# linto-ai/ssak

Hardware: AMD Instinct MI355X
Metric: utterances/sec (16 kHz, 10 s) Wav2Vec2-base CTC train step (higher is better)
Workload: dtype bf16; 1 GPU; Wav2Vec2-base CTC fine-tune step, bf16, synthetic 10 s @16 kHz utterances (BASELINE.json configs[1]; DP over xGMI for n_gpus>1 = configs[2]); per_gpu_batch=32, global_batch=32, samples_per_utt=160000, frames=499, frozen_feature_encoder=True, regularisers=script defaults (dropout/layerdrop/specaugment on), parallelism=dp1

## Files before the change

### ssak_amd/csrc/attention.hip

```cpp
#include <utility>

#include "kernels.h"

namespace {

constexpr int HD = 64;
constexpr int KT = 64;
constexpr int TILE = 2;
constexpr int TILE_BYTES = KT * HD * 2;
typedef __attribute__((address_space(3))) void lds_void_t;
typedef __attribute__((address_space(3))) s16x4 lds_s16x4_t;
typedef __attribute__((ext_vector_type(8))) short s16x8_t;
typedef __attribute__((ext_vector_type(4))) uint32_t u32x4_t;

struct AttnParams {
  const bf16* qkv;
  bf16* ctx;
  float* lse;
  const int32_t* klens;
  const bf16* dctx;
  float* delta;
  bf16* dqkv;
  float* bias_part;
  int B, F, nh, H, Fp;
  float scale;
  uint64_t seed;
  uint32_t stream, thresh16;
  float drop_scale;
};

__device__ __forceinline__ float shfl_xor_f(float v, int m) { return __shfl_xor(v, m, 64); }
__device__ __forceinline__ float softmax_offset(float v, float slack) {
  float x = v, y = v;
  asm volatile("s_nop 1\n\tv_permlane16_swap_b32 %0, %1" : "+v"(x), "+v"(y));
  float pm;
  asm("v_max_f32 %0, %1, %2" : "=v"(pm) : "v"(x), "v"(y));
  float a = pm, b = pm;
  asm volatile("s_nop 1\n\tv_permlane32_swap_b32 %0, %1" : "+v"(a), "+v"(b));
  float all;
  asm("v_max_f32 %0, %1, %2" : "=v"(all) : "v"(a), "v"(b));
  float g0 = x, g2 = x;
  asm volatile("s_nop 1\n\tv_permlane32_swap_b32 %0, %1" : "+v"(g0), "+v"(g2));
  float r;
  asm("v_max_f32 %0, %1, %2" : "=v"(r) : "v"(g0), "v"(all - slack));
  return r;
}
__device__ __forceinline__ float max2_nc(float a, float b) {
  float d;
  asm("v_max_f32 %0, %1, %2" : "=v"(d) : "v"(a), "v"(b));
  return d;
}
__device__ __forceinline__ float max3_nc(float a, float b, float c) {
  float d;
  asm("v_max3_f32 %0, %1, %2, %3" : "=v"(d) : "v"(a), "v"(b), "v"(c));
  return d;
}
__device__ __forceinline__ int opaque_s(int v) {
  asm volatile("" : "+s"(v));
  return v;
}

__device__ __forceinline__ uint32_t drop_rowseed(const AttnParams& p, int b, int h, int q) {
  return drop_rowkey(p.seed, p.stream, (uint64_t)((uint32_t)(b * p.nh + h) * (uint32_t)p.F + (uint32_t)min(q, p.F - 1)));
}
__device__ __forceinline__ void fill_colmul(uint32_t* cmt, int n) {
  for (int k = threadIdx.x; k < n; k += 256) cmt[k] = drop_colmul((uint32_t)k);
}

#ifdef ATT_OLD_DUAL
__device__ __forceinline__ int dual_swz(int r) {
  const int x = (r >> 1) & 7;
  return ((x << 1) & 7) | (x >> 2);
}
#else
__device__ __forceinline__ int dual_swz(int r) { return r & 6; }
#endif
__device__ __forceinline__ void dma_tile(__amdgpu_buffer_rsrc_t rsrc, char* lds_tile, uint32_t col_byte, long ld_bytes,
                                         int row0, int nrows_total, int image , int wave, int lane) {
#pragma unroll
  for (int j = 0; j < 2; ++j) {
    const int S = (wave * 2 + j) * 64 + lane;
    const int r = S >> 3, pc = S & 7;
    const int c = image == 2 ? (pc ^ dual_swz(r)) : image == 1 ? (pc ^ (r & 6)) : (pc ^ ((r >> 1) & 7));
    const int gr = row0 + r;
    const uint32_t off = gr < nrows_total ? (uint32_t)((long)gr * ld_bytes + col_byte + c * 16) : 0x80000000u;
    __builtin_amdgcn_raw_ptr_buffer_load_lds(rsrc, (lds_void_t*)(lds_tile + (wave * 2 + j) * 1024), 16, off, 0, 0, 0);
  }
}

struct DmaOff {
  uint32_t o[2];
};
__device__ __forceinline__ DmaOff dma_offsets(uint32_t col_byte, long ld_bytes, int image, int wave, int lane) {
  DmaOff d;
#pragma unroll
  for (int j = 0; j < 2; ++j) {
    const int S = (wave * 2 + j) * 64 + lane;
    const int r = S >> 3, pc = S & 7;
    const int c = image == 2 ? (pc ^ dual_swz(r)) : image == 1 ? (pc ^ (r & 6)) : (pc ^ ((r >> 1) & 7));
    d.o[j] = (uint32_t)((long)r * ld_bytes + col_byte + c * 16);
  }
  return d;
}
__device__ __forceinline__ __amdgpu_buffer_rsrc_t rsrc_rows(const void* base, long ld_bytes, int row0, int nrows) {
  const long skip = (long)row0 * ld_bytes;
  return __builtin_amdgcn_make_buffer_rsrc((void*)((const char*)base + skip), 0, (int)((long)max(nrows - row0, 0) * ld_bytes), 0x00020000);
}
__device__ __forceinline__ void dma_tile_at(__amdgpu_buffer_rsrc_t rsrc, char* lds_tile, const DmaOff& d, int wave) {
#pragma unroll
  for (int j = 0; j < 2; ++j)
    __builtin_amdgcn_raw_ptr_buffer_load_lds(rsrc, (lds_void_t*)(lds_tile + (wave * 2 + j) * 1024), 16, d.o[j], 0, 0, 0);
}

__device__ __forceinline__ bf16x8 frag_rows(const char* tile, int sub, int kk, int lane) {
  const int r = 16 * sub + (lane & 15);
  const int c = kk * 4 + (lane >> 4);
  return *reinterpret_cast<const bf16x8*>(tile + r * 128 + ((c ^ ((r >> 1) & 7)) << 4));
}
__device__ __forceinline__ bf16x8 frag_cols_perm(const char* tile, int ci, int rbase, int lane) {
  const int g = lane >> 4, q4 = (lane >> 2) & 3, p4 = lane & 3;
  const int r = rbase + 4 * g + q4;
  const int ch = 2 * ci + (p4 >> 1);
  const char* a = tile + r * 128 + ((ch ^ (r & 6)) << 4) + (p4 & 1) * 8;
  const s16x4 lo = __builtin_amdgcn_ds_read_tr16_b64_v4i16((lds_s16x4_t*)(a));
  const s16x4 hi = __builtin_amdgcn_ds_read_tr16_b64_v4i16((lds_s16x4_t*)(a + 16 * 128));
  s16x8_t v = __builtin_shufflevector(lo, hi, 0, 1, 2, 3, 4, 5, 6, 7);
  return __builtin_bit_cast(bf16x8, v);
}

__device__ __forceinline__ bf16x8 frag_rows_d(const char* tile, int sub, int kk, int lane) {
  const int r = 16 * sub + (lane & 15);
  const int c = kk * 4 + (lane >> 4);
  return *reinterpret_cast<const bf16x8*>(tile + r * 128 + ((c ^ dual_swz(r)) << 4));
}
__device__ __forceinline__ bf16x8 frag_cols_perm_d(const char* tile, int ci, int rbase, int lane) {
  const int g = lane >> 4, q4 = (lane >> 2) & 3, p4 = lane & 3;
  const int r = rbase + 4 * g + q4;
  const int ch = 2 * ci + (p4 >> 1);
  const char* a = tile + r * 128 + ((ch ^ dual_swz(r)) << 4) + (p4 & 1) * 8;
  const s16x4 lo = __builtin_amdgcn_ds_read_tr16_b64_v4i16((lds_s16x4_t*)(a));
  const s16x4 hi = __builtin_amdgcn_ds_read_tr16_b64_v4i16((lds_s16x4_t*)(a + 16 * 128));
  s16x8_t v = __builtin_shufflevector(lo, hi, 0, 1, 2, 3, 4, 5, 6, 7);
  return __builtin_bit_cast(bf16x8, v);
}

__device__ __forceinline__ bf16x8 pack_p(const f32x4& a, const f32x4& b) {
  const bf16x4 lo = __builtin_convertvector(a, bf16x4), hi = __builtin_convertvector(b, bf16x4);
  return __builtin_shufflevector(lo, hi, 0, 1, 2, 3, 4, 5, 6, 7);
}

__device__ __forceinline__ bf16x8 load_row_frag(const bf16* base, long ld, int row, int nrows, int kk, int lane) {
  bf16x8 z = {};
  if (row >= nrows) return z;
  return *reinterpret_cast<const bf16x8*>(base + (long)row * ld + 32 * kk + 8 * (lane >> 4));
}

struct AttnBlock {
  int b, h, blk;
};
__device__ __forceinline__ AttnBlock attn_block() {
  const int nblk = gridDim.x, nh = gridDim.y, nbh = gridDim.y * gridDim.z;
  AttnBlock r;
  if ((nbh & 7) != 0) {
    r.b = blockIdx.z, r.h = blockIdx.y, r.blk = blockIdx.x;
    return r;
  }
  const int L = blockIdx.x + nblk * (blockIdx.y + nh * blockIdx.z);
  const int xcd = L & 7, j = L >> 3;
  const int bh = (j / nblk) * 8 + xcd;
  r.blk = j % nblk;
  r.b = bh / nh;
  r.h = bh % nh;
  return r;
}

template <int NS>
__device__ __forceinline__ void bias_partial(float (&cs)[NS][4][4], char* smem, float* dst , int set_stride,
                                             int wave, int lane) {
#pragma unroll
  for (int s = 0; s < NS; ++s)
#pragma unroll
    for (int i = 0; i < 4; ++i)
#pragma unroll
      for (int r = 0; r < 4; ++r) {
        float v = cs[s][i][r];
        v += dpp_f<0xB1, 0xf>(0.f, v);
        v += dpp_f<0x4E, 0xf>(0.f, v);
        v += dpp_f<0x141, 0xf>(0.f, v);
        v += dpp_f<0x140, 0xf>(0.f, v);
        cs[s][i][r] = v;
      }
  float* red = reinterpret_cast<float*>(smem);
  lds_barrier();
  if ((lane & 15) == 0) {
#pragma unroll
    for (int s = 0; s < NS; ++s)
#pragma unroll
      for (int i = 0; i < 4; ++i)
        *reinterpret_cast<f32x4*>(red + (s * 4 + wave) * HD + 16 * i + 4 * (lane >> 4)) = (f32x4){cs[s][i][0], cs[s][i][1], cs[s][i][2], cs[s][i][3]};
  }
  lds_barrier();
  if (wave < NS) {
    const float* rs = red + wave * 4 * HD;
    dst[wave * set_stride + lane] = (rs[lane] + rs[HD + lane]) + (rs[2 * HD + lane] + rs[3 * HD + lane]);
  }
}
__device__ __forceinline__ float bf16_round(float v) { return (float)(bf16)v; }

typedef __attribute__((ext_vector_type(2))) float f32x2;

template <bool DROP, int NQS>
__global__ __launch_bounds__(256) void attn_fwd_kernel(const AttnParams p) {
  extern __shared__ __attribute__((aligned(16))) char smem[];
  const int lane = threadIdx.x & 63, wave = __builtin_amdgcn_readfirstlane(threadIdx.x >> 6);
  const AttnBlock ab = attn_block();
  const int b = ab.b, h = ab.h, q0 = ab.blk * (64 * NQS);
  const int F = p.F, H = p.H;
  const long ld = 3L * H;
  const bf16* base = p.qkv + (long)b * F * ld;
  const int kl = p.klens ? min(max(p.klens[b], 0), F) : F;
  const int nkt = (kl + KT - 1) / KT;
  __amdgpu_buffer_rsrc_t rsrc = __builtin_amdgcn_make_buffer_rsrc((void*)base, 0, (int)((long)F * ld * 2), 0x00020000);
  const uint32_t kcol = (uint32_t)((H + h * HD) * 2), vcol = (uint32_t)((2 * H + h * HD) * 2);

  int qrow[NQS];
  bf16x8 qf[NQS][2];
#pragma unroll
  for (int qs = 0; qs < NQS; ++qs) {
    qrow[qs] = q0 + 16 * NQS * wave + 16 * qs + (lane & 15);
#pragma unroll
    for (int kk = 0; kk < 2; ++kk) qf[qs][kk] = load_row_frag(base + h * HD, ld, qrow[qs], F, kk, lane);
  }
  float m_run[NQS], l_run[NQS];
#pragma unroll
  for (int qs = 0; qs < NQS; ++qs) {
    m_run[qs] = -INFINITY;
    l_run[qs] = 0.f;
  }
  const float c2 = p.scale * 1.4426950408889634f;
  const float slack = 12.f / c2;
  const uint32_t thi = p.thresh16 << 16;
  uint32_t rowseed[NQS];
#pragma unroll
  for (int qs = 0; qs < NQS; ++qs) rowseed[qs] = drop_rowseed(p, b, h, qrow[qs]);
  const uint32_t* cmt = reinterpret_cast<const uint32_t*>(smem + 2 * 2 * TILE_BYTES);
  if (DROP) fill_colmul(reinterpret_cast<uint32_t*>(smem + 2 * 2 * TILE_BYTES), nkt * KT);
  f32x4 oacc[NQS][4];
#pragma unroll
  for (int qs = 0; qs < NQS; ++qs)
#pragma unroll
    for (int i = 0; i < 4; ++i) oacc[qs][i] = (f32x4){0.f, 0.f, 0.f, 0.f};

  const DmaOff koff = dma_offsets(kcol, ld * 2, 0, wave, lane), voff = dma_offsets(vcol, ld * 2, 1, wave, lane);
  if (nkt > 0) {
    dma_tile_at(rsrc, smem, koff, wave);
    dma_tile_at(rsrc, smem + TILE_BYTES, voff, wave);
  }
  const int g = lane >> 4;
  for (int kt = 0; kt < nkt; ++kt) {
    const int cur = kt & 1;
    __builtin_amdgcn_s_waitcnt(0x0f70);
    __syncthreads();
    if (kt + 1 < nkt) {
      const __amdgpu_buffer_rsrc_t rn = rsrc_rows(base, ld * 2, (kt + 1) * KT, F);
      dma_tile_at(rn, smem + (cur ^ 1) * 2 * TILE_BYTES, koff, wave);
      dma_tile_at(rn, smem + (cur ^ 1) * 2 * TILE_BYTES + TILE_BYTES, voff, wave);
    }
    const char* kt_lds = smem + cur * 2 * TILE_BYTES;
    const char* vt_lds = kt_lds + TILE_BYTES;
    const int k0 = kt * KT;
    f32x4 s[NQS][4];
#pragma unroll
    for (int ks = 0; ks < 4; ++ks) {
      const bf16x8 ka = frag_rows(kt_lds, ks, 0, lane), kb = frag_rows(kt_lds, ks, 1, lane);
#pragma unroll
      for (int qs = 0; qs < NQS; ++qs) {
        f32x4 a = {0.f, 0.f, 0.f, 0.f};
        a = __builtin_amdgcn_mfma_f32_16x16x32_bf16(ka, qf[qs][0], a, 0, 0, 0);
        a = __builtin_amdgcn_mfma_f32_16x16x32_bf16(kb, qf[qs][1], a, 0, 0, 0);
        s[qs][ks] = a;
      }
    }
    bf16x8 pb[NQS][2];
    const bool edge = k0 + KT > kl;
    u32x4_t cm[4];
    if (DROP) {
#pragma unroll
      for (int ks = 0; ks < 4; ++ks) cm[ks] = *reinterpret_cast<const u32x4_t*>(cmt + k0 + 16 * ks + 4 * g);
    }
#pragma unroll
    for (int qs = 0; qs < NQS; ++qs) {
      if (edge) {
        const int tl = opaque_s(kl) - k0 - 4 * g;
#pragma unroll
        for (int ks = 0; ks < 4; ++ks)
#pragma unroll
          for (int r = 0; r < 4; ++r)
            if (16 * ks + r >= tl) s[qs][ks][r] = -INFINITY;
      }
      float mx = max3_nc(s[qs][0][0], s[qs][0][1], s[qs][0][2]);
      mx = max3_nc(mx, s[qs][0][3], s[qs][1][0]);
#pragma unroll
      for (int ks = 1; ks < 4; ++ks) {
        mx = max3_nc(mx, s[qs][ks][1], s[qs][ks][2]);
        if (ks < 3)
          mx = max3_nc(mx, s[qs][ks][3], s[qs][ks + 1][0]);
        else
          mx = max2_nc(mx, s[qs][ks][3]);
      }
      mx = softmax_offset(mx, slack);
      const float m_new = max2_nc(m_run[qs], mx);
      const float mc = m_new * c2;
      const float alpha = __builtin_amdgcn_exp2f(fmaf(m_run[qs], c2, -mc));
      f32x2 rs2 = {0.f, 0.f};
      const f32x2 c2v = {c2, c2}, mcv = {-mc, -mc};
#pragma unroll
      for (int ks = 0; ks < 4; ++ks) {
#pragma unroll
        for (int r2 = 0; r2 < 4; r2 += 2) {
          const f32x2 a = (f32x2){s[qs][ks][r2], s[qs][ks][r2 + 1]} * c2v + mcv;
          f32x2 e = {__builtin_amdgcn_exp2f(a[0]), __builtin_amdgcn_exp2f(a[1])};
          rs2 += e;
          if (DROP) {
            e[0] = drop_keep(rowseed[qs], cm[ks][r2], thi) ? e[0] : 0.f;
            e[1] = drop_keep(rowseed[qs], cm[ks][r2 + 1], thi) ? e[1] : 0.f;
          }
          s[qs][ks][r2] = e[0];
          s[qs][ks][r2 + 1] = e[1];
        }
      }
      l_run[qs] = l_run[qs] * alpha + (rs2[0] + rs2[1]);
      m_run[qs] = m_new;
      if (__builtin_amdgcn_ballot_w64(alpha != 1.f)) {
#pragma unroll
        for (int i = 0; i < 4; ++i) oacc[qs][i] *= alpha;
      }
      pb[qs][0] = pack_p(s[qs][0], s[qs][1]);
      pb[qs][1] = pack_p(s[qs][2], s[qs][3]);
    }
#pragma unroll
    for (int t2 = 0; t2 < 2; ++t2)
#pragma unroll
      for (int i = 0; i < 4; ++i) {
        const bf16x8 va = frag_cols_perm(vt_lds, i, 32 * t2, lane);
#pragma unroll
        for (int qs = 0; qs < NQS; ++qs) oacc[qs][i] = __builtin_amdgcn_mfma_f32_16x16x32_bf16(va, pb[qs][t2], oacc[qs][i], 0, 0, 0);
      }
  }
#pragma unroll
  for (int qs = 0; qs < NQS; ++qs) {
    const int q = qrow[qs];
    float lsum = l_run[qs];
    lsum += shfl_xor_f(lsum, 16);
    lsum += shfl_xor_f(lsum, 32);
    if (q >= F) continue;
    const float inv = lsum > 0.f ? p.drop_scale / lsum : 0.f;
    if (g == 0 && p.lse)
      p.lse[((long)b * p.nh + h) * F + q] = lsum > 0.f ? m_run[qs] * p.scale + __logf(lsum) : -INFINITY;
    bf16* dst = p.ctx + ((long)b * F + q) * H + h * HD + 4 * g;
#pragma unroll
    for (int i = 0; i < 4; ++i) {
      const bf16x4 o = {(bf16)(oacc[qs][i][0] * inv), (bf16)(oacc[qs][i][1] * inv), (bf16)(oacc[qs][i][2] * inv),
                        (bf16)(oacc[qs][i][3] * inv)};
      *reinterpret_cast<bf16x4*>(dst + 16 * i) = o;
    }
  }
}

__global__ __launch_bounds__(256) void attn_delta_kernel(const bf16* __restrict__ dctx, const bf16* __restrict__ ctx,
                                                         float* __restrict__ delta, int B, int F, int nh, int H) {
  const int lane = threadIdx.x & 63;
  const long row = (long)blockIdx.x * 4 + (threadIdx.x >> 6);
  if (row >= (long)B * F) return;
  const int b = (int)(row / F), q = (int)(row % F);
  for (int h = 0; h < nh; ++h) {
    const long o = row * H + h * HD + lane;
    float v = (float)dctx[o] * (float)ctx[o];
    v = wave_sum(v);
    if (lane == 0) delta[((long)b * nh + h) * F + q] = v;
  }
}

template <bool DROP, int NQS>
__global__ __launch_bounds__(256, 2) void attn_bwd_dq_kernel(const AttnParams p) {
  extern __shared__ __attribute__((aligned(16))) char smem[];
  const int lane = threadIdx.x & 63, wave = __builtin_amdgcn_readfirstlane(threadIdx.x >> 6);
  const AttnBlock ab = attn_block();
  const int b = ab.b, h = ab.h, q0 = ab.blk * (64 * NQS);
  const int F = p.F, H = p.H;
  const long ld = 3L * H;
  const bf16* base = p.qkv + (long)b * F * ld;
  const int kl = p.klens ? min(max(p.klens[b], 0), F) : F;
  const int nkt = (kl + KT - 1) / KT;
  const uint32_t kcol = (uint32_t)((H + h * HD) * 2), vcol = (uint32_t)((2 * H + h * HD) * 2);
  const int g = lane >> 4;
  int qrow[NQS];
  bf16x8 qf[NQS][2], dof[NQS][2];
  float lse[NQS], dl[NQS], lse2[NQS];
  uint32_t rowbase[NQS];
  const float c2 = p.scale * 1.4426950408889634f;
  const uint32_t thi = p.thresh16 << 16;
#pragma unroll
  for (int qs = 0; qs < NQS; ++qs) {
    qrow[qs] = q0 + 16 * NQS * wave + 16 * qs + (lane & 15);
    rowbase[qs] = drop_rowseed(p, b, h, qrow[qs]);
    const int qc = min(qrow[qs], F - 1);
    lse[qs] = p.lse[((long)b * p.nh + h) * F + qc];
    lse2[qs] = lse[qs] > -INFINITY ? fmaf(lse[qs], 1.4426950408889634f, -__log2f(p.scale * p.drop_scale)) : INFINITY;
    float part = 0.f;
#pragma unroll
    for (int kk = 0; kk < 2; ++kk) {
      qf[qs][kk] = load_row_frag(base + h * HD, ld, qrow[qs], F, kk, lane);
      dof[qs][kk] = load_row_frag(p.dctx + (long)b * F * H + h * HD, H, qrow[qs], F, kk, lane);
      const bf16x8 of = load_row_frag(p.ctx + (long)b * F * H + h * HD, H, qrow[qs], F, kk, lane);
#pragma unroll
      for (int j = 0; j < 8; ++j) part = fmaf((float)dof[qs][kk][j], (float)of[j], part);
    }
    part += shfl_xor_f(part, 16);
    part += shfl_xor_f(part, 32);
    dl[qs] = part / p.drop_scale;
    if (g == 0 && qrow[qs] < F) p.delta[((long)b * p.nh + h) * F + qrow[qs]] = part;
  }
  f32x4 dq[NQS][4];
#pragma unroll
  for (int qs = 0; qs < NQS; ++qs)
#pragma unroll
    for (int i = 0; i < 4; ++i) dq[qs][i] = (f32x4){0.f, 0.f, 0.f, 0.f};
  const uint32_t* cmt = reinterpret_cast<const uint32_t*>(smem + 2 * 2 * TILE_BYTES);
  if (DROP) fill_colmul(reinterpret_cast<uint32_t*>(smem + 2 * 2 * TILE_BYTES), nkt * KT);
  const DmaOff koff = dma_offsets(kcol, ld * 2, 2, wave, lane), voff = dma_offsets(vcol, ld * 2, 2, wave, lane);
  auto issue = [&](int kt, int stage) {
    char* s0 = smem + stage * 2 * TILE_BYTES;
    const __amdgpu_buffer_rsrc_t rn = rsrc_rows(base, ld * 2, kt * KT, F);
    dma_tile_at(rn, s0, koff, wave);
    dma_tile_at(rn, s0 + TILE_BYTES, voff, wave);
  };
  if (nkt > 0) issue(0, 0);
  for (int kt = 0; kt < nkt; ++kt) {
    const int cur = kt & 1;
    __builtin_amdgcn_s_waitcnt(0x0f70);
    __syncthreads();
    if (kt + 1 < nkt) issue(kt + 1, cur ^ 1);
    const char* k_rows = smem + cur * 2 * TILE_BYTES;
    const char* k_tr = k_rows;
    const char* v_rows = k_rows + TILE_BYTES;
    const int k0 = kt * KT;
    const bool edge = k0 + KT > kl;
#pragma unroll
    for (int t2 = 0; t2 < 2; ++t2) {
      bf16x8 dsb[NQS];
      {
        f32x4 s[NQS][2], dp[NQS][2];
#pragma unroll
        for (int kh = 0; kh < 2; ++kh) {
          const int ks = 2 * t2 + kh;
          const bf16x8 ka = frag_rows_d(k_rows, ks, 0, lane), kb = frag_rows_d(k_rows, ks, 1, lane);
          const bf16x8 va = frag_rows_d(v_rows, ks, 0, lane), vb = frag_rows_d(v_rows, ks, 1, lane);
#pragma unroll
          for (int qs = 0; qs < NQS; ++qs) {
            f32x4 a = {0.f, 0.f, 0.f, 0.f}, c = {0.f, 0.f, 0.f, 0.f};
            a = __builtin_amdgcn_mfma_f32_16x16x32_bf16(ka, qf[qs][0], a, 0, 0, 0);
            a = __builtin_amdgcn_mfma_f32_16x16x32_bf16(kb, qf[qs][1], a, 0, 0, 0);
            c = __builtin_amdgcn_mfma_f32_16x16x32_bf16(va, dof[qs][0], c, 0, 0, 0);
            c = __builtin_amdgcn_mfma_f32_16x16x32_bf16(vb, dof[qs][1], c, 0, 0, 0);
            s[qs][kh] = a;
            dp[qs][kh] = c;
          }
        }
        if (edge) {
          const int tl = opaque_s(kl) - k0 - 4 * g;
#pragma unroll
          for (int qs = 0; qs < NQS; ++qs)
#pragma unroll
            for (int kh = 0; kh < 2; ++kh)
#pragma unroll
              for (int r = 0; r < 4; ++r)
                if (16 * (2 * t2 + kh) + r >= tl) s[qs][kh][r] = -INFINITY;
        }
        u32x4_t cm[2];
        if (DROP) {
#pragma unroll
          for (int kh = 0; kh < 2; ++kh) cm[kh] = *reinterpret_cast<const u32x4_t*>(cmt + k0 + 16 * (2 * t2 + kh) + 4 * g);
        }
#pragma unroll
        for (int qs = 0; qs < NQS; ++qs) {
          const f32x2 c2v = {c2, c2}, lscv = {-lse2[qs], -lse2[qs]}, ndlv = {-dl[qs], -dl[qs]};
#pragma unroll
          for (int kh = 0; kh < 2; ++kh)
#pragma unroll
            for (int r2 = 0; r2 < 4; r2 += 2) {
              f32x2 d = {dp[qs][kh][r2], dp[qs][kh][r2 + 1]};
              if (DROP) {
                d[0] = drop_keep(rowbase[qs], cm[kh][r2], thi) ? d[0] : 0.f;
                d[1] = drop_keep(rowbase[qs], cm[kh][r2 + 1], thi) ? d[1] : 0.f;
              }
              const f32x2 a = (f32x2){s[qs][kh][r2], s[qs][kh][r2 + 1]} * c2v + lscv;
              const f32x2 pv = {__builtin_amdgcn_exp2f(a[0]), __builtin_amdgcn_exp2f(a[1])};
              const f32x2 ds2 = __builtin_elementwise_fma(pv, d, pv * ndlv);
              s[qs][kh][r2] = ds2[0];
              s[qs][kh][r2 + 1] = ds2[1];
            }
          dsb[qs] = pack_p(s[qs][0], s[qs][1]);
        }
      }
#pragma unroll
      for (int i = 0; i < 4; ++i) {
        const bf16x8 ka = frag_cols_perm_d(k_tr, i, 32 * t2, lane);
#pragma unroll
        for (int qs = 0; qs < NQS; ++qs) dq[qs][i] = __builtin_amdgcn_mfma_f32_16x16x32_bf16(ka, dsb[qs], dq[qs][i], 0, 0, 0);
      }
    }
  }
#pragma unroll
  for (int qs = 0; qs < NQS; ++qs) {
    const int q = qrow[qs];
    if (q >= F) continue;
    bf16* dst = p.dqkv + ((long)b * F + q) * ld + h * HD + 4 * g;
#pragma unroll
    for (int i = 0; i < 4; ++i) {
      const bf16x4 o = {(bf16)dq[qs][i][0], (bf16)dq[qs][i][1], (bf16)dq[qs][i][2], (bf16)dq[qs][i][3]};
      *reinterpret_cast<bf16x4*>(dst + 16 * i) = o;
    }
  }
  if (p.bias_part) {
    float cs[1][4][4];
#pragma unroll
    for (int i = 0; i < 4; ++i)
#pragma unroll
      for (int r = 0; r < 4; ++r) {
        float v = 0.f;
#pragma unroll
        for (int qs = 0; qs < NQS; ++qs) v += qrow[qs] < F ? bf16_round(dq[qs][i][r]) : 0.f;
        cs[0][i][r] = v;
      }
    bias_partial<1>(cs, smem, p.bias_part + ((long)b * gridDim.x + ab.blk) * ld + h * HD, 0, wave, lane);
  }
}

template <bool DROP, int NKS, bool MASK>
__global__ __launch_bounds__(256, 2) void attn_bwd_dkv_kernel(const AttnParams p) {
  extern __shared__ __attribute__((aligned(16))) char smem[];
  const int lane = threadIdx.x & 63, wave = __builtin_amdgcn_readfirstlane(threadIdx.x >> 6);
  const AttnBlock ab = attn_block();
  const int b = ab.b, h = ab.h, key0 = ab.blk * (64 * NKS);
  const int F = p.F, H = p.H;
  const long ld = 3L * H;
  const bf16* base = p.qkv + (long)b * F * ld;
  const int kl = p.klens ? min(max(p.klens[b], 0), F) : F;
  const int nqt = (F + KT - 1) / KT;
  const uint32_t qcol = (uint32_t)(h * HD * 2);
  const int g = lane >> 4;
  float* stat = reinterpret_cast<float*>(smem + 2 * 2 * TILE_BYTES);
  int krow[NKS];
  bf16x8 kf[NKS][2], vf[NKS][2];
#pragma unroll
  for (int ks = 0; ks < NKS; ++ks) {
    krow[ks] = key0 + 16 * NKS * wave + 16 * ks + (lane & 15);
#pragma unroll
    for (int kk = 0; kk < 2; ++kk) {
      kf[ks][kk] = load_row_frag(base + H + h * HD, ld, krow[ks], F, kk, lane);
      vf[ks][kk] = load_row_frag(base + 2 * H + h * HD, ld, krow[ks], F, kk, lane);
    }
  }
  const float c2 = p.scale * 1.4426950408889634f;
  const float log2scale = __log2f(p.scale * p.drop_scale);
  const float inv_drop_scale = 1.f / p.drop_scale;
  const uint32_t thi = p.thresh16 << 16;
  uint32_t cmk[NKS];
#pragma unroll
  for (int ks = 0; ks < NKS; ++ks) cmk[ks] = DROP ? drop_colmul((uint32_t)krow[ks]) : 1u;
  f32x4 sinit[NKS];
#pragma unroll
  for (int ks = 0; ks < NKS; ++ks) {
    const float v = krow[ks] < kl ? 0.f : -3.0e38f;
    sinit[ks] = (f32x4){v, v, v, v};
  }
  f32x4 dk[NKS][4], dv[NKS][4];
#pragma unroll
  for (int ks = 0; ks < NKS; ++ks)
#pragma unroll
    for (int i = 0; i < 4; ++i) {
      dk[ks][i] = (f32x4){0.f, 0.f, 0.f, 0.f};
      dv[ks][i] = (f32x4){0.f, 0.f, 0.f, 0.f};
    }
  const DmaOff qoff = dma_offsets(qcol, ld * 2, 2, wave, lane), dooff = dma_offsets(qcol, (long)H * 2, 2, wave, lane);
  const bf16* const do_base = p.dctx + (long)b * F * H;
  auto issue = [&](int qt, int stage) {
    char* s0 = smem + stage * 2 * TILE_BYTES;
    dma_tile_at(rsrc_rows(base, ld * 2, qt * KT, F), s0, qoff, wave);
    dma_tile_at(rsrc_rows(do_base, (long)H * 2, qt * KT, F), s0 + TILE_BYTES, dooff, wave);
  };
  float st_l = -INFINITY, st_d = 0.f;
  int st_q = 0;
  auto load_stat = [&](int qt) {
    if (threadIdx.x < KT) {
      st_q = qt * KT + threadIdx.x;
      const long o = ((long)b * p.nh + h) * F + min(st_q, F - 1);
      st_l = p.lse[o];
      st_d = p.delta[o];
    }
  };
  auto write_stat = [&](int stage) {
    if (threadIdx.x < KT) {
      const float ls = st_q < F ? st_l : -INFINITY;
      stat[stage * 3 * KT + threadIdx.x] = ls > -INFINITY ? fmaf(ls, 1.4426950408889634f, -log2scale) : INFINITY;
      stat[stage * 3 * KT + KT + threadIdx.x] = st_q < F ? st_d * inv_drop_scale : 0.f;
      reinterpret_cast<uint32_t*>(stat)[stage * 3 * KT + 2 * KT + threadIdx.x] = drop_rowseed(p, b, h, st_q);
    }
  };
  load_stat(0);
  write_stat(0);
  if (nqt > 1) load_stat(1);
  issue(0, 0);
  for (int qt = 0; qt < nqt; ++qt) {
    const int cur = qt & 1;
    __builtin_amdgcn_s_waitcnt(0x0f70);
    __syncthreads();
    if (qt + 1 < nqt) {
      write_stat(cur ^ 1);
      if (qt + 2 < nqt) load_stat(qt + 2);
      issue(qt + 1, cur ^ 1);
    }
    const char* q_rows = smem + cur * 2 * TILE_BYTES;
    const char* q_tr = q_rows;
    const char* do_rows = q_rows + TILE_BYTES;
    const char* do_tr = do_rows;
    const float* lse_s = stat + cur * 3 * KT;
    const float* dl_s = lse_s + KT;
    const uint32_t* seed_s = reinterpret_cast<const uint32_t*>(lse_s + 2 * KT);
#pragma unroll
    for (int t2 = 0; t2 < 2; ++t2) {
      bf16x8 pdb[NKS], dsb[NKS];
      {
        f32x4 s[NKS][2], dp[NKS][2];
#pragma unroll
        for (int qh = 0; qh < 2; ++qh) {
          const int qsb = 2 * t2 + qh;
          const bf16x8 qa = frag_rows_d(q_rows, qsb, 0, lane), qb = frag_rows_d(q_rows, qsb, 1, lane);
          const bf16x8 da = frag_rows_d(do_rows, qsb, 0, lane), db = frag_rows_d(do_rows, qsb, 1, lane);
#pragma unroll
          for (int ks = 0; ks < NKS; ++ks) {
            f32x4 a = {0.f, 0.f, 0.f, 0.f}, c = {0.f, 0.f, 0.f, 0.f};
            if (MASK) a = sinit[ks];
            a = __builtin_amdgcn_mfma_f32_16x16x32_bf16(qa, kf[ks][0], a, 0, 0, 0);
            a = __builtin_amdgcn_mfma_f32_16x16x32_bf16(qb, kf[ks][1], a, 0, 0, 0);
            c = __builtin_amdgcn_mfma_f32_16x16x32_bf16(da, vf[ks][0], c, 0, 0, 0);
            c = __builtin_amdgcn_mfma_f32_16x16x32_bf16(db, vf[ks][1], c, 0, 0, 0);
            s[ks][qh] = a;
            dp[ks][qh] = c;
          }
        }
#pragma unroll
        for (int qh = 0; qh < 2; ++qh) {
          u32x4_t rk = {1u, 1u, 1u, 1u};
          if (DROP) rk = *reinterpret_cast<const u32x4_t*>(seed_s + 16 * (2 * t2 + qh) + 4 * g);
#pragma unroll
          for (int r = 0; r < 4; r += 2) {
            const int ql = 16 * (2 * t2 + qh) + 4 * g + r;
            const f32x2 c2v = {c2, c2}, lscv = {-lse_s[ql], -lse_s[ql + 1]}, ndlv = {-dl_s[ql], -dl_s[ql + 1]};
#pragma unroll
            for (int ks = 0; ks < NKS; ++ks) {
              const f32x2 a = (f32x2){s[ks][qh][r], s[ks][qh][r + 1]} * c2v + lscv;
              const f32x2 pr = {__builtin_amdgcn_exp2f(a[0]), __builtin_amdgcn_exp2f(a[1])};
              const f32x2 dpv = {dp[ks][qh][r], dp[ks][qh][r + 1]};
              f32x2 pd = pr;
              if (DROP) {
#pragma unroll
                for (int e = 0; e < 2; ++e) pd[e] = drop_keep(rk[r + e], cmk[ks], thi) ? pd[e] : 0.f;
              }
              const f32x2 ds2 = __builtin_elementwise_fma(pd, dpv, pr * ndlv);
              s[ks][qh][r] = pd[0];
              s[ks][qh][r + 1] = pd[1];
              dp[ks][qh][r] = ds2[0];
              dp[ks][qh][r + 1] = ds2[1];
            }
          }
        }
#pragma unroll
        for (int ks = 0; ks < NKS; ++ks) {
          pdb[ks] = pack_p(s[ks][0], s[ks][1]);
          dsb[ks] = pack_p(dp[ks][0], dp[ks][1]);
        }
      }
#pragma unroll
      for (int i = 0; i < 4; ++i) {
        const bf16x8 doa = frag_cols_perm_d(do_tr, i, 32 * t2, lane);
        const bf16x8 qa = frag_cols_perm_d(q_tr, i, 32 * t2, lane);
#pragma unroll
        for (int ks = 0; ks < NKS; ++ks) {
          dv[ks][i] = __builtin_amdgcn_mfma_f32_16x16x32_bf16(doa, pdb[ks], dv[ks][i], 0, 0, 0);
          dk[ks][i] = __builtin_amdgcn_mfma_f32_16x16x32_bf16(qa, dsb[ks], dk[ks][i], 0, 0, 0);
        }
      }
    }
  }
  const float inv_scale = 1.f / p.scale;
#pragma unroll
  for (int ks = 0; ks < NKS; ++ks) {
    const int key = krow[ks];
    if (key >= F) continue;
    bf16* dkd = p.dqkv + ((long)b * F + key) * ld + H + h * HD + 4 * g;
    bf16* dvd = dkd + H;
#pragma unroll
    for (int i = 0; i < 4; ++i) {
      const bf16x4 a = {(bf16)dk[ks][i][0], (bf16)dk[ks][i][1], (bf16)dk[ks][i][2], (bf16)dk[ks][i][3]};
      const bf16x4 c = {(bf16)(dv[ks][i][0] * inv_scale), (bf16)(dv[ks][i][1] * inv_scale), (bf16)(dv[ks][i][2] * inv_scale),
                        (bf16)(dv[ks][i][3] * inv_scale)};
      *reinterpret_cast<bf16x4*>(dkd + 16 * i) = a;
      *reinterpret_cast<bf16x4*>(dvd + 16 * i) = c;
    }
  }
  if (p.bias_part) {
    float cs[2][4][4];
#pragma unroll
    for (int i = 0; i < 4; ++i)
#pragma unroll
      for (int r = 0; r < 4; ++r) {
        float vk = 0.f, vv = 0.f;
#pragma unroll
        for (int ks = 0; ks < NKS; ++ks) {
          vk += krow[ks] < F ? bf16_round(dk[ks][i][r]) : 0.f;
          vv += krow[ks] < F ? bf16_round(dv[ks][i][r] * inv_scale) : 0.f;
        }
        cs[0][i][r] = vk;
        cs[1][i][r] = vv;
      }
    bias_partial<2>(cs, smem, p.bias_part + ((long)b * gridDim.x + ab.blk) * ld + H + h * HD, H, wave, lane);
  }
}


AttnParams make_params(const bf16* qkv, bf16* ctx, float* lse, const int32_t* klens, const bf16* dctx, float* delta, bf16* dqkv,
                       int B, int F, int nh, int H, const DropSpec& drop) {
  AttnParams p;
  p.qkv = qkv;
  p.ctx = ctx;
  p.lse = lse;
  p.klens = klens;
  p.dctx = dctx;
  p.delta = delta;
  p.dqkv = dqkv;
  p.bias_part = nullptr;
  p.B = B;
  p.F = F;
  p.nh = nh;
  p.H = H;
  p.Fp = (F + 7) & ~7;
  p.scale = 1.f / sqrtf((float)HD);
  p.seed = drop.seed;
  p.stream = drop.stream;
  p.thresh16 = drop.p > 0.f ? (uint32_t)fminf(65535.f, roundf(drop.p * 65536.f)) : 0u;
  p.drop_scale = p.thresh16 ? 1.f / (1.f - (float)p.thresh16 / 65536.f) : 1.f;
  return p;
}

}

bool k_attention_supported(int H, int nh) { return nh > 0 && H / nh == HD && H % nh == 0; }

int k_attention_fwd(const bf16* qkv, bf16* ctx, float* lse, const int32_t* klens, int B, int F, int nh, int H,
                    const DropSpec& drop, hipStream_t st) {
  SSAK_REQUIRE(k_attention_supported(H, nh), "attention: fused kernels are built for head_dim 64 (got %d)", nh ? H / nh : 0);
  SSAK_REQUIRE((long)F * 3 * H * 2 < 2000000000L, "attention: one utterance of q|k|v must span < 2 GB");
  const AttnParams p = make_params(qkv, ctx, lse, klens, nullptr, nullptr, nullptr, B, F, nh, H, drop);
  ProfScope prof_scope(PROF_ATTN_FWD, 4.0 * B * nh * (double)F * F * HD, st);
  SSAK_REQUIRE(!p.thresh16 || F <= DROP_TABLE_N, "attention: dropout is built for at most %d frames", DROP_TABLE_N);
  const int cm_lds = p.thresh16 ? ssak_cdiv(F, KT) * KT * 4 : 0;
  static bool fwd_attr_done = false;
  if (!fwd_attr_done) {
    SSAK_HIP(hipFuncSetAttribute((const void*)attn_fwd_kernel<true, 2>, hipFuncAttributeMaxDynamicSharedMemorySize, 2 * 2 * TILE_BYTES + DROP_TABLE_N * 4));
    fwd_attr_done = true;
  }
#define ATT_LAUNCH_FWD(D) attn_fwd_kernel<D, TILE><<<dim3(ssak_cdiv(F, 64 * TILE), nh, B), 256, 2 * 2 * TILE_BYTES + cm_lds, st>>>(p)
  if (p.thresh16) ATT_LAUNCH_FWD(true); else ATT_LAUNCH_FWD(false);
#undef ATT_LAUNCH_FWD
  SSAK_LAUNCH_CHECK();
  return SSAK_OK;
}

size_t k_attention_bwd_bias_floats(int B, int F, int H) {
  return (size_t)B * ssak_cdiv(F, 64 * TILE) * 3 * H;
}

int k_attention_bwd(const bf16* qkv, const bf16* ctx, const float* lse, const int32_t* klens, const bf16* dctx, float* delta,
                    bf16* dqkv, int B, int F, int nh, int H, const DropSpec& drop, int mode, hipStream_t st, float* bias_part,
                    float* bias_grad) {
  SSAK_REQUIRE(k_attention_supported(H, nh), "attention: fused kernels are built for head_dim 64 (got %d)", nh ? H / nh : 0);
  SSAK_REQUIRE(mode == SSAK_ATTN_BWD_DEFAULT || mode == SSAK_ATTN_BWD_TWO_KERNEL,
               "attention_bwd: mode %d (0 / 1 = two kernels; the single-pass form, 2, was removed in ABI 400)", mode);
  SSAK_REQUIRE(!bias_part == !bias_grad, "attention_bwd: bias partials need both pointers");
  AttnParams p = make_params(qkv, const_cast<bf16*>(ctx), const_cast<float*>(lse), klens, dctx, delta, dqkv, B, F, nh, H, drop);
  p.bias_part = bias_part;
  ProfScope prof_scope(PROF_ATTN_BWD, 8.0 * B * nh * (double)F * F * HD, st);
  SSAK_REQUIRE(!p.thresh16 || F <= DROP_TABLE_N, "attention: dropout is built for at most %d frames", DROP_TABLE_N);
  const int cm_lds = p.thresh16 ? ssak_cdiv(F, KT) * KT * 4 : 0;
  static bool dq_attr_done = false;
  if (!dq_attr_done) {
    SSAK_HIP(hipFuncSetAttribute((const void*)attn_bwd_dq_kernel<true, 2>, hipFuncAttributeMaxDynamicSharedMemorySize, 2 * 2 * TILE_BYTES + DROP_TABLE_N * 4));
    dq_attr_done = true;
  }
#define ATT_LAUNCH_DQ(D) attn_bwd_dq_kernel<D, TILE><<<dim3(ssak_cdiv(F, 64 * TILE), nh, B), 256, 2 * 2 * TILE_BYTES + cm_lds, st>>>(p)
  if (p.thresh16) ATT_LAUNCH_DQ(true); else ATT_LAUNCH_DQ(false);
#undef ATT_LAUNCH_DQ
  SSAK_LAUNCH_CHECK();
  constexpr int dkv_lds = 2 * 2 * TILE_BYTES + 2 * 3 * KT * 4;
  static bool attr_done = false;
  if (!attr_done) {
#define ATT_DKV_ATTR(D, K) SSAK_HIP(hipFuncSetAttribute((const void*)attn_bwd_dkv_kernel<D, TILE, K>, hipFuncAttributeMaxDynamicSharedMemorySize, dkv_lds))
    ATT_DKV_ATTR(true, true); ATT_DKV_ATTR(false, true); ATT_DKV_ATTR(true, false); ATT_DKV_ATTR(false, false);
#undef ATT_DKV_ATTR
    attr_done = true;
  }
#define ATT_LAUNCH_DKV(D)                                                                                             \
  do {                                                                                                                \
    if (klens) attn_bwd_dkv_kernel<D, TILE, true><<<dim3(ssak_cdiv(F, 64 * TILE), nh, B), 256, dkv_lds, st>>>(p);    \
    else attn_bwd_dkv_kernel<D, TILE, false><<<dim3(ssak_cdiv(F, 64 * TILE), nh, B), 256, dkv_lds, st>>>(p);         \
  } while (0)
  if (p.thresh16) ATT_LAUNCH_DKV(true); else ATT_LAUNCH_DKV(false);
#undef ATT_LAUNCH_DKV
  SSAK_LAUNCH_CHECK();
  if (bias_part) {
    const int slots = B * ssak_cdiv(F, 64 * TILE);
    if (!(g_reduce_sink && g_reduce_sink->push(bias_part, 3L * H, slots, 3 * H, bias_grad))) {
      const int rc = k_colsum_rows(bias_part, slots, 3 * H, bias_grad, st);
      if (rc != SSAK_OK) return rc;
    }
  }
  return SSAK_OK;
}

extern "C" int ssak_attention_fwd(const void* qkv, void* ctx, float* lse, const int32_t* klens, int B, int F, int nh, int H,
                                  float drop_p, uint64_t seed, uint32_t stream_id, void* stream) {
  SSAK_REQUIRE(qkv && ctx && lse, "attention_fwd: null pointer");
  DropSpec d;
  d.p = drop_p;
  d.seed = seed;
  d.stream = stream_id;
  return k_attention_fwd((const bf16*)qkv, (bf16*)ctx, lse, klens, B, F, nh, H, d, (hipStream_t)stream);
}

extern "C" int ssak_attention_bwd(const void* qkv, const void* ctx, const float* lse, const int32_t* klens, const void* dctx,
                                  float* delta, void* dqkv, int B, int F, int nh, int H, float drop_p, uint64_t seed,
                                  uint32_t stream_id, int mode, void* stream) {
  SSAK_REQUIRE(qkv && ctx && lse && dctx && delta && dqkv, "attention_bwd: null pointer");
  DropSpec d;
  d.p = drop_p;
  d.seed = seed;
  d.stream = stream_id;
  return k_attention_bwd((const bf16*)qkv, (const bf16*)ctx, lse, klens, (const bf16*)dctx, delta, (bf16*)dqkv, B, F, nh, H, d, mode,
                         (hipStream_t)stream);
}

extern "C" size_t ssak_attention_bwd_bias_workspace_bytes(int B, int F, int H) {
  return (size_t)B * ssak_cdiv(F > 0 ? F : 1, 64) * 3 * (H > 0 ? H : 0) * sizeof(float);
}
extern "C" int ssak_attention_bwd_bias(const void* qkv, const void* ctx, const float* lse, const int32_t* klens, const void* dctx,
                                       float* delta, void* dqkv, float* bias_grad, int B, int F, int nh, int H, float drop_p,
                                       uint64_t seed, uint32_t stream_id, void* workspace, size_t workspace_bytes, void* stream) {
  SSAK_REQUIRE(qkv && ctx && lse && dctx && delta && dqkv && bias_grad && workspace, "attention_bwd_bias: null pointer");
  SSAK_REQUIRE(workspace_bytes >= ssak_attention_bwd_bias_workspace_bytes(B, F, H), "attention_bwd_bias: workspace too small");
  DropSpec d;
  d.p = drop_p;
  d.seed = seed;
  d.stream = stream_id;
  return k_attention_bwd((const bf16*)qkv, (const bf16*)ctx, lse, klens, (const bf16*)dctx, delta, (bf16*)dqkv, B, F, nh, H, d,
                         SSAK_ATTN_BWD_DEFAULT, (hipStream_t)stream, (float*)workspace, bias_grad);
}
```

Before: 2247 utterances/sec.

## Rewrite attention forward with 32x32x16 MFMA tiles and a matching LDS swizzle

```diff
diff --git a/ssak_amd/csrc/attention.hip b/ssak_amd/csrc/attention.hip
--- a/ssak_amd/csrc/attention.hip
+++ b/ssak_amd/csrc/attention.hip
@@ -30,19 +30,15 @@
 };
 
 __device__ __forceinline__ float shfl_xor_f(float v, int m) { return __shfl_xor(v, m, 64); }
-__device__ __forceinline__ float softmax_offset(float v, float slack) {
-  float x = v, y = v;
-  asm volatile("s_nop 1\n\tv_permlane16_swap_b32 %0, %1" : "+v"(x), "+v"(y));
-  float pm;
-  asm("v_max_f32 %0, %1, %2" : "=v"(pm) : "v"(x), "v"(y));
-  float a = pm, b = pm;
+__device__ __forceinline__ float softmax_offset(float g0, float v, float slack) {
+  float x = g0, y = g0;
+  asm volatile("s_nop 1\n\tv_permlane32_swap_b32 %0, %1" : "+v"(x), "+v"(y));
+  float a = v, b = v;
   asm volatile("s_nop 1\n\tv_permlane32_swap_b32 %0, %1" : "+v"(a), "+v"(b));
   float all;
   asm("v_max_f32 %0, %1, %2" : "=v"(all) : "v"(a), "v"(b));
-  float g0 = x, g2 = x;
-  asm volatile("s_nop 1\n\tv_permlane32_swap_b32 %0, %1" : "+v"(g0), "+v"(g2));
   float r;
-  asm("v_max_f32 %0, %1, %2" : "=v"(r) : "v"(g0), "v"(all - slack));
+  asm("v_max_f32 %0, %1, %2" : "=v"(r) : "v"(x), "v"(all - slack));
   return r;
 }
 __device__ __forceinline__ float max2_nc(float a, float b) {
@@ -55,6 +51,12 @@
   asm("v_max3_f32 %0, %1, %2, %3" : "=v"(d) : "v"(a), "v"(b), "v"(c));
   return d;
 }
+__device__ __forceinline__ float max16_nc(const float (&v)[16]) {
+  float m = max3_nc(v[0], v[1], v[2]);
+#pragma unroll
+  for (int i = 3; i < 15; i += 2) m = max3_nc(m, v[i], v[i + 1]);
+  return max2_nc(m, v[15]);
+}
 __device__ __forceinline__ int opaque_s(int v) {
   asm volatile("" : "+s"(v));
   return v;
@@ -75,29 +77,18 @@
 #else
 __device__ __forceinline__ int dual_swz(int r) { return r & 6; }
 #endif
-__device__ __forceinline__ void dma_tile(__amdgpu_buffer_rsrc_t rsrc, char* lds_tile, uint32_t col_byte, long ld_bytes,
-                                         int row0, int nrows_total, int image , int wave, int lane) {
+__device__ __forceinline__ int swz32(int r) { return ((r & 2) << 1) | ((r >> 2) & 1) | ((r >> 3) & 2); }
+
+struct DmaOff {
+  uint32_t o[2];
+};
+__device__ __forceinline__ DmaOff dma_offsets(uint32_t col_byte, long ld_bytes, int image , int wave, int lane) {
+  DmaOff d;
 #pragma unroll
   for (int j = 0; j < 2; ++j) {
     const int S = (wave * 2 + j) * 64 + lane;
     const int r = S >> 3, pc = S & 7;
-    const int c = image == 2 ? (pc ^ dual_swz(r)) : image == 1 ? (pc ^ (r & 6)) : (pc ^ ((r >> 1) & 7));
-    const int gr = row0 + r;
-    const uint32_t off = gr < nrows_total ? (uint32_t)((long)gr * ld_bytes + col_byte + c * 16) : 0x80000000u;
-    __builtin_amdgcn_raw_ptr_buffer_load_lds(rsrc, (lds_void_t*)(lds_tile + (wave * 2 + j) * 1024), 16, off, 0, 0, 0);
-  }
-}
-
-struct DmaOff {
-  uint32_t o[2];
-};
-__device__ __forceinline__ DmaOff dma_offsets(uint32_t col_byte, long ld_bytes, int image, int wave, int lane) {
-  DmaOff d;
-#pragma unroll
-  for (int j = 0; j < 2; ++j) {
-    const int S = (wave * 2 + j) * 64 + lane;
-    const int r = S >> 3, pc = S & 7;
-    const int c = image == 2 ? (pc ^ dual_swz(r)) : image == 1 ? (pc ^ (r & 6)) : (pc ^ ((r >> 1) & 7));
+    const int c = pc ^ (image == 3 ? swz32(r) : dual_swz(r));
     d.o[j] = (uint32_t)((long)r * ld_bytes + col_byte + c * 16);
   }
   return d;
@@ -110,22 +101,6 @@
 #pragma unroll
   for (int j = 0; j < 2; ++j)
     __builtin_amdgcn_raw_ptr_buffer_load_lds(rsrc, (lds_void_t*)(lds_tile + (wave * 2 + j) * 1024), 16, d.o[j], 0, 0, 0);
-}
-
-__device__ __forceinline__ bf16x8 frag_rows(const char* tile, int sub, int kk, int lane) {
-  const int r = 16 * sub + (lane & 15);
-  const int c = kk * 4 + (lane >> 4);
-  return *reinterpret_cast<const bf16x8*>(tile + r * 128 + ((c ^ ((r >> 1) & 7)) << 4));
-}
-__device__ __forceinline__ bf16x8 frag_cols_perm(const char* tile, int ci, int rbase, int lane) {
-  const int g = lane >> 4, q4 = (lane >> 2) & 3, p4 = lane & 3;
-  const int r = rbase + 4 * g + q4;
-  const int ch = 2 * ci + (p4 >> 1);
-  const char* a = tile + r * 128 + ((ch ^ (r & 6)) << 4) + (p4 & 1) * 8;
-  const s16x4 lo = __builtin_amdgcn_ds_read_tr16_b64_v4i16((lds_s16x4_t*)(a));
-  const s16x4 hi = __builtin_amdgcn_ds_read_tr16_b64_v4i16((lds_s16x4_t*)(a + 16 * 128));
-  s16x8_t v = __builtin_shufflevector(lo, hi, 0, 1, 2, 3, 4, 5, 6, 7);
-  return __builtin_bit_cast(bf16x8, v);
 }
 
 __device__ __forceinline__ bf16x8 frag_rows_d(const char* tile, int sub, int kk, int lane) {
@@ -144,6 +119,21 @@
   return __builtin_bit_cast(bf16x8, v);
 }
 
+__device__ __forceinline__ bf16x8 frag_rows32(const char* tile, int kb, int kd, int lane) {
+  const int r = 32 * kb + (lane & 31);
+  const int c = 2 * kd + (lane >> 5);
+  return *reinterpret_cast<const bf16x8*>(tile + r * 128 + ((c ^ swz32(r)) << 4));
+}
+__device__ __forceinline__ bf16x8 frag_cols_perm32(const char* tile, int db, int rbase, int lane) {
+  const int q4 = (lane >> 2) & 3, p4 = lane & 3;
+  const int r = rbase + 4 * (lane >> 5) + q4;
+  const int ch = 4 * db + 2 * ((lane >> 4) & 1) + (p4 >> 1);
+  const char* a = tile + r * 128 + ((ch ^ swz32(r)) << 4) + (p4 & 1) * 8;
+  const s16x4 lo = __builtin_amdgcn_ds_read_tr16_b64_v4i16((lds_s16x4_t*)(a));
+  const s16x4 hi = __builtin_amdgcn_ds_read_tr16_b64_v4i16((lds_s16x4_t*)(a + 8 * 128));
+  s16x8_t v = __builtin_shufflevector(lo, hi, 0, 1, 2, 3, 4, 5, 6, 7);
+  return __builtin_bit_cast(bf16x8, v);
+}
 __device__ __forceinline__ bf16x8 pack_p(const f32x4& a, const f32x4& b) {
   const bf16x4 lo = __builtin_convertvector(a, bf16x4), hi = __builtin_convertvector(b, bf16x4);
   return __builtin_shufflevector(lo, hi, 0, 1, 2, 3, 4, 5, 6, 7);
@@ -209,12 +199,13 @@
 
 typedef __attribute__((ext_vector_type(2))) float f32x2;
 
-template <bool DROP, int NQS>
-__global__ __launch_bounds__(256) void attn_fwd_kernel(const AttnParams p) {
+typedef __attribute__((ext_vector_type(16))) float f32x16;
+template <bool DROP>
+__global__ __launch_bounds__(256, 3) void attn_fwd_kernel(const AttnParams p) {
   extern __shared__ __attribute__((aligned(16))) char smem[];
   const int lane = threadIdx.x & 63, wave = __builtin_amdgcn_readfirstlane(threadIdx.x >> 6);
   const AttnBlock ab = attn_block();
-  const int b = ab.b, h = ab.h, q0 = ab.blk * (64 * NQS);
+  const int b = ab.b, h = ab.h, q0 = ab.blk * (64 * TILE);
   const int F = p.F, H = p.H;
   const long ld = 3L * H;
   const bf16* base = p.qkv + (long)b * F * ld;
@@ -222,41 +213,33 @@
   const int nkt = (kl + KT - 1) / KT;
   __amdgpu_buffer_rsrc_t rsrc = __builtin_amdgcn_make_buffer_rsrc((void*)base, 0, (int)((long)F * ld * 2), 0x00020000);
   const uint32_t kcol = (uint32_t)((H + h * HD) * 2), vcol = (uint32_t)((2 * H + h * HD) * 2);
-
-  int qrow[NQS];
-  bf16x8 qf[NQS][2];
-#pragma unroll
-  for (int qs = 0; qs < NQS; ++qs) {
-    qrow[qs] = q0 + 16 * NQS * wave + 16 * qs + (lane & 15);
-#pragma unroll
-    for (int kk = 0; kk < 2; ++kk) qf[qs][kk] = load_row_frag(base + h * HD, ld, qrow[qs], F, kk, lane);
-  }
-  float m_run[NQS], l_run[NQS];
-#pragma unroll
-  for (int qs = 0; qs < NQS; ++qs) {
-    m_run[qs] = -INFINITY;
-    l_run[qs] = 0.f;
-  }
+  const int hh = lane >> 5;
+
+  const int qrow = q0 + 32 * wave + (lane & 31);
+  bf16x8 qf[4];
+#pragma unroll
+  for (int kd = 0; kd < 4; ++kd) {
+    bf16x8 z = {};
+    qf[kd] = qrow < F ? *reinterpret_cast<const bf16x8*>(base + h * HD + (long)qrow * ld + 16 * kd + 8 * hh) : z;
+  }
+  float m_run = -INFINITY, l_run = 0.f;
   const float c2 = p.scale * 1.4426950408889634f;
   const float slack = 12.f / c2;
   const uint32_t thi = p.thresh16 << 16;
-  uint32_t rowseed[NQS];
-#pragma unroll
-  for (int qs = 0; qs < NQS; ++qs) rowseed[qs] = drop_rowseed(p, b, h, qrow[qs]);
+  const uint32_t rowseed = drop_rowseed(p, b, h, qrow);
   const uint32_t* cmt = reinterpret_cast<const uint32_t*>(smem + 2 * 2 * TILE_BYTES);
   if (DROP) fill_colmul(reinterpret_cast<uint32_t*>(smem + 2 * 2 * TILE_BYTES), nkt * KT);
-  f32x4 oacc[NQS][4];
-#pragma unroll
-  for (int qs = 0; qs < NQS; ++qs)
-#pragma unroll
-    for (int i = 0; i < 4; ++i) oacc[qs][i] = (f32x4){0.f, 0.f, 0.f, 0.f};
-
-  const DmaOff koff = dma_offsets(kcol, ld * 2, 0, wave, lane), voff = dma_offsets(vcol, ld * 2, 1, wave, lane);
+  f32x16 oacc[2];
+#pragma unroll
+  for (int db = 0; db < 2; ++db)
+#pragma unroll
+    for (int i = 0; i < 16; ++i) oacc[db][i] = 0.f;
+
+  const DmaOff koff = dma_offsets(kcol, ld * 2, 3, wave, lane), voff = dma_offsets(vcol, ld * 2, 3, wave, lane);
   if (nkt > 0) {
     dma_tile_at(rsrc, smem, koff, wave);
     dma_tile_at(rsrc, smem + TILE_BYTES, voff, wave);
   }
-  const int g = lane >> 4;
   for (int kt = 0; kt < nkt; ++kt) {
     const int cur = kt & 1;
     __builtin_amdgcn_s_waitcnt(0x0f70);
@@ -269,102 +252,90 @@
     const char* kt_lds = smem + cur * 2 * TILE_BYTES;
     const char* vt_lds = kt_lds + TILE_BYTES;
     const int k0 = kt * KT;
-    f32x4 s[NQS][4];
-#pragma unroll
-    for (int ks = 0; ks < 4; ++ks) {
-      const bf16x8 ka = frag_rows(kt_lds, ks, 0, lane), kb = frag_rows(kt_lds, ks, 1, lane);
-#pragma unroll
-      for (int qs = 0; qs < NQS; ++qs) {
-        f32x4 a = {0.f, 0.f, 0.f, 0.f};
-        a = __builtin_amdgcn_mfma_f32_16x16x32_bf16(ka, qf[qs][0], a, 0, 0, 0);
-        a = __builtin_amdgcn_mfma_f32_16x16x32_bf16(kb, qf[qs][1], a, 0, 0, 0);
-        s[qs][ks] = a;
-      }
-    }
-    bf16x8 pb[NQS][2];
+    f32x16 s[2];
+#pragma unroll
+    for (int kb = 0; kb < 2; ++kb) {
+      f32x16 a;
+#pragma unroll
+      for (int i = 0; i < 16; ++i) a[i] = 0.f;
+#pragma unroll
+      for (int kd = 0; kd < 4; ++kd) a = __builtin_amdgcn_mfma_f32_32x32x16_bf16(frag_rows32(kt_lds, kb, kd, lane), qf[kd], a, 0, 0, 0);
+      s[kb] = a;
+    }
     const bool edge = k0 + KT > kl;
-    u32x4_t cm[4];
-    if (DROP) {
-#pragma unroll
-      for (int ks = 0; ks < 4; ++ks) cm[ks] = *reinterpret_cast<const u32x4_t*>(cmt + k0 + 16 * ks + 4 * g);
-    }
-#pragma unroll
-    for (int qs = 0; qs < NQS; ++qs) {
-      if (edge) {
-        const int tl = opaque_s(kl) - k0 - 4 * g;
-#pragma unroll
-        for (int ks = 0; ks < 4; ++ks)
-#pragma unroll
-          for (int r = 0; r < 4; ++r)
-            if (16 * ks + r >= tl) s[qs][ks][r] = -INFINITY;
-      }
-      float mx = max3_nc(s[qs][0][0], s[qs][0][1], s[qs][0][2]);
-      mx = max3_nc(mx, s[qs][0][3], s[qs][1][0]);
-#pragma unroll
-      for (int ks = 1; ks < 4; ++ks) {
-        mx = max3_nc(mx, s[qs][ks][1], s[qs][ks][2]);
-        if (ks < 3)
-          mx = max3_nc(mx, s[qs][ks][3], s[qs][ks + 1][0]);
-        else
-          mx = max2_nc(mx, s[qs][ks][3]);
-      }
-      mx = softmax_offset(mx, slack);
-      const float m_new = max2_nc(m_run[qs], mx);
-      const float mc = m_new * c2;
-      const float alpha = __builtin_amdgcn_exp2f(fmaf(m_run[qs], c2, -mc));
-      f32x2 rs2 = {0.f, 0.f};
-      const f32x2 c2v = {c2, c2}, mcv = {-mc, -mc};
-#pragma unroll
-      for (int ks = 0; ks < 4; ++ks) {
-#pragma unroll
-        for (int r2 = 0; r2 < 4; r2 += 2) {
-          const f32x2 a = (f32x2){s[qs][ks][r2], s[qs][ks][r2 + 1]} * c2v + mcv;
-          f32x2 e = {__builtin_amdgcn_exp2f(a[0]), __builtin_amdgcn_exp2f(a[1])};
-          rs2 += e;
-          if (DROP) {
-            e[0] = drop_keep(rowseed[qs], cm[ks][r2], thi) ? e[0] : 0.f;
-            e[1] = drop_keep(rowseed[qs], cm[ks][r2 + 1], thi) ? e[1] : 0.f;
-          }
-          s[qs][ks][r2] = e[0];
-          s[qs][ks][r2 + 1] = e[1];
-        }
-      }
-      l_run[qs] = l_run[qs] * alpha + (rs2[0] + rs2[1]);
-      m_run[qs] = m_new;
-      if (__builtin_amdgcn_ballot_w64(alpha != 1.f)) {
-#pragma unroll
-        for (int i = 0; i < 4; ++i) oacc[qs][i] *= alpha;
-      }
-      pb[qs][0] = pack_p(s[qs][0], s[qs][1]);
-      pb[qs][1] = pack_p(s[qs][2], s[qs][3]);
-    }
-#pragma unroll
-    for (int t2 = 0; t2 < 2; ++t2)
-#pragma unroll
-      for (int i = 0; i < 4; ++i) {
-        const bf16x8 va = frag_cols_perm(vt_lds, i, 32 * t2, lane);
-#pragma unroll
-        for (int qs = 0; qs < NQS; ++qs) oacc[qs][i] = __builtin_amdgcn_mfma_f32_16x16x32_bf16(va, pb[qs][t2], oacc[qs][i], 0, 0, 0);
-      }
-  }
-#pragma unroll
-  for (int qs = 0; qs < NQS; ++qs) {
-    const int q = qrow[qs];
-    float lsum = l_run[qs];
-    lsum += shfl_xor_f(lsum, 16);
-    lsum += shfl_xor_f(lsum, 32);
-    if (q >= F) continue;
-    const float inv = lsum > 0.f ? p.drop_scale / lsum : 0.f;
-    if (g == 0 && p.lse)
-      p.lse[((long)b * p.nh + h) * F + q] = lsum > 0.f ? m_run[qs] * p.scale + __logf(lsum) : -INFINITY;
-    bf16* dst = p.ctx + ((long)b * F + q) * H + h * HD + 4 * g;
-#pragma unroll
-    for (int i = 0; i < 4; ++i) {
-      const bf16x4 o = {(bf16)(oacc[qs][i][0] * inv), (bf16)(oacc[qs][i][1] * inv), (bf16)(oacc[qs][i][2] * inv),
-                        (bf16)(oacc[qs][i][3] * inv)};
-      *reinterpret_cast<bf16x4*>(dst + 16 * i) = o;
-    }
-  }
+    if (edge) {
+      const int tl = opaque_s(kl) - k0 - 4 * hh;
+#pragma unroll
+      for (int kb = 0; kb < 2; ++kb)
+#pragma unroll
+        for (int i = 0; i < 16; ++i)
+          if (32 * kb + 8 * (i >> 2) + (i & 3) >= tl) s[kb][i] = -INFINITY;
+    }
+    float sg[2][16];
+#pragma unroll
+    for (int kb = 0; kb < 2; ++kb)
+#pragma unroll
+      for (int i = 0; i < 16; ++i) sg[(i >> 2) & 1][8 * kb + 4 * (i >> 3) + (i & 3)] = s[kb][i];
+    const float mg = max16_nc(sg[0]);
+    const float mx = softmax_offset(mg, max2_nc(mg, max16_nc(sg[1])), slack);
+    const float m_new = max2_nc(m_run, mx);
+    const float mc = m_new * c2;
+    const float alpha = __builtin_amdgcn_exp2f(fmaf(m_run, c2, -mc));
+    f32x2 rs2 = {0.f, 0.f};
+    const f32x2 c2v = {c2, c2}, mcv = {-mc, -mc};
+#pragma unroll
+    for (int kb = 0; kb < 2; ++kb) {
+      u32x4_t cm[4];
+      if (DROP) {
+#pragma unroll
+        for (int t = 0; t < 4; ++t) cm[t] = *reinterpret_cast<const u32x4_t*>(cmt + k0 + 32 * kb + 8 * t + 4 * hh);
+      }
+#pragma unroll
+      for (int i = 0; i < 16; i += 2) {
+        const f32x2 a = (f32x2){s[kb][i], s[kb][i + 1]} * c2v + mcv;
+        f32x2 e = {__builtin_amdgcn_exp2f(a[0]), __builtin_amdgcn_exp2f(a[1])};
+        rs2 += e;
+        if (DROP) {
+          e[0] = drop_keep(rowseed, cm[i >> 2][i & 3], thi) ? e[0] : 0.f;
+          e[1] = drop_keep(rowseed, cm[i >> 2][(i & 3) + 1], thi) ? e[1] : 0.f;
+        }
+        s[kb][i] = e[0];
+        s[kb][i + 1] = e[1];
+      }
+    }
+    l_run = l_run * alpha + (rs2[0] + rs2[1]);
+    m_run = m_new;
+    if (__builtin_amdgcn_ballot_w64(alpha != 1.f)) {
+#pragma unroll
+      for (int db = 0; db < 2; ++db) oacc[db] *= alpha;
+    }
+#pragma unroll
+    for (int kb = 0; kb < 2; ++kb)
+#pragma unroll
+      for (int st = 0; st < 2; ++st) {
+        const f32x4 lo = {s[kb][8 * st], s[kb][8 * st + 1], s[kb][8 * st + 2], s[kb][8 * st + 3]};
+        const f32x4 hi = {s[kb][8 * st + 4], s[kb][8 * st + 5], s[kb][8 * st + 6], s[kb][8 * st + 7]};
+        const bf16x8 pb = pack_p(lo, hi);
+#pragma unroll
+        for (int db = 0; db < 2; ++db)
+          oacc[db] = __builtin_amdgcn_mfma_f32_32x32x16_bf16(frag_cols_perm32(vt_lds, db, 32 * kb + 16 * st, lane), pb, oacc[db], 0, 0, 0);
+      }
+  }
+  float lsum = l_run;
+  lsum += shfl_xor_f(lsum, 32);
+  if (qrow >= F) return;
+  const float inv = lsum > 0.f ? p.drop_scale / lsum : 0.f;
+  if (hh == 0 && p.lse)
+    p.lse[((long)b * p.nh + h) * F + qrow] = lsum > 0.f ? m_run * p.scale + __logf(lsum) : -INFINITY;
+  bf16* dst = p.ctx + ((long)b * F + qrow) * H + h * HD + 4 * hh;
+#pragma unroll
+  for (int db = 0; db < 2; ++db)
+#pragma unroll
+    for (int t = 0; t < 4; ++t) {
+      const bf16x4 o = {(bf16)(oacc[db][4 * t] * inv), (bf16)(oacc[db][4 * t + 1] * inv), (bf16)(oacc[db][4 * t + 2] * inv),
+                        (bf16)(oacc[db][4 * t + 3] * inv)};
+      *reinterpret_cast<bf16x4*>(dst + 32 * db + 8 * t) = o;
+    }
 }
 
 __global__ __launch_bounds__(256) void attn_delta_kernel(const bf16* __restrict__ dctx, const bf16* __restrict__ ctx,
@@ -768,10 +739,10 @@
   const int cm_lds = p.thresh16 ? ssak_cdiv(F, KT) * KT * 4 : 0;
   static bool fwd_attr_done = false;
   if (!fwd_attr_done) {
-    SSAK_HIP(hipFuncSetAttribute((const void*)attn_fwd_kernel<true, 2>, hipFuncAttributeMaxDynamicSharedMemorySize, 2 * 2 * TILE_BYTES + DROP_TABLE_N * 4));
+    SSAK_HIP(hipFuncSetAttribute((const void*)attn_fwd_kernel<true>, hipFuncAttributeMaxDynamicSharedMemorySize, 2 * 2 * TILE_BYTES + DROP_TABLE_N * 4));
     fwd_attr_done = true;
   }
-#define ATT_LAUNCH_FWD(D) attn_fwd_kernel<D, TILE><<<dim3(ssak_cdiv(F, 64 * TILE), nh, B), 256, 2 * 2 * TILE_BYTES + cm_lds, st>>>(p)
+#define ATT_LAUNCH_FWD(D) attn_fwd_kernel<D><<<dim3(ssak_cdiv(F, 64 * TILE), nh, B), 256, 2 * 2 * TILE_BYTES + cm_lds, st>>>(p)
   if (p.thresh16) ATT_LAUNCH_FWD(true); else ATT_LAUNCH_FWD(false);
 #undef ATT_LAUNCH_FWD
   SSAK_LAUNCH_CHECK();
```

After: 2248 utterances/sec (median of 5 runs). Within noise of the previous version (+0.0%).
